# wadx2019/rpo

Measured on AMD Instinct MI355X. Metric: env-steps/sec (whole node), SafeCartpole-v0 (CartSafe-v0) RPODDPG, rollout + one batch-256 constrained policy update per vector step, higher is better.
Workload: dtype f32; 1 GPU; CartSafe-v0 RPODDPG, 4096 vectorised envs per MI355X, scripts/cart_exp.py hyper-parameters, update batch 256 every vector step (reference cadence), replay capacity 20000 per env; envs_per_gpu=4096, global_envs=4096, update_batch=256, hip_graph=True, training_batch_projection=row-wise, rccl_ranks=0, collectives_in_graph=False, graphs_replayed_on_all_ranks=True, graph_capture_fell_back_to_eager=False

## Files before the change

### include/rpo_hip.h

```cpp
#ifndef RPO_HIP_H
#define RPO_HIP_H

#ifdef __cplusplus
extern "C" {
#endif

#define RPO_ABI_VERSION 6

#define RPO_ERR_ARG (-1)
#define RPO_ERR_NULL (-2)

#define RPO_CART_STATE_DIM 6
#define RPO_CART_ACTION_DIM 2
#define RPO_CART_INEQ 6
#define RPO_CART_ROW 24
#define RPO_CART_RING 32
#define RPO_CART_CONSTS_LEN 35

#define RPO_PEND_INTERNAL_DIM 4
#define RPO_PEND_OBS_DIM 5
#define RPO_PEND_ACTION_DIM 2
#define RPO_PEND_ROW 16
#define RPO_PEND_RING 16

// ... 355 lines not shown
int rpo_evopf_reset(int n_envs, float* state, int* ep_len, float* ep_ret, const unsigned* ep_count,
                    const float* consts_dev, unsigned long long seed, unsigned env_id_base, void* stream);

int rpo_evopf_step(int n_envs, float* state, const float* action, int* ep_len, float* ep_ret, unsigned* ep_count,
                   float* rows, long long cap_steps, float* stats, int stats_cap, long long* ctrl, int max_episode_steps,
                   int auto_reset, float viol_thresh, const float* consts_dev, unsigned long long seed,
                   unsigned env_id_base, void* stream);

int rpo_evopf_act_project(int n, const float* state, int state_stride, const float* ap_raw, const float* noise, float* action, int* iters,
                          int noise_mode, int ap_is_raw, float eps_start, float eps_end, float eps_decay, int max_steps,
                          float corr_lr, float corr_eps, float corr_momentum, float newton_tol, int newton_max_iters,
                          const float* consts_dev, unsigned long long seed, unsigned env_id_base, const long long* ctrl,
                          float* stats, int stats_cap, void* stream);

int rpo_evopf_tanh_box_bwd(int n, const float* state, int state_stride, const float* raw, const float* noise,
                           float eps_start, float eps_end, float eps_decay, const long long* ctrl, const float* dap,
                           float* dout, const float* consts_dev, void* stream);

int rpo_evopf_gauss_head(int n, const float* state, int state_stride, const float* raw, const float* eps, int deterministic,
                         float* ap_out, float* logp_out, const float* consts_dev, void* stream);
int rpo_evopf_gauss_head_bwd(int n, const float* state, int state_stride, const float* raw, const float* eps,
                             const float* dap, float dlogp, float* draw, const float* consts_dev, void* stream);

int rpo_evopf_complete_bwd(int n, const float* action, const float* grad_action, const float* grad_action_b, const float* grad_action2,
                           float* grad_ap, const float* consts_dev, void* stream);

int rpo_evopf_resid(int n, const float* state, int state_stride, const float* action, float* eq_out, float* ineq_out,
                    const float* consts_dev, void* stream);

int rpo_evopf_ineq_partial_grad(int n, const float* state, int state_stride, const float* action, float* step_out, const float* consts_dev,
                                void* stream);

int rpo_evopf_eq_vjp(int n, const float* action, const float* grad_eq, float* grad_action, int autograd_sign,
                     const float* consts_dev, void* stream);

int rpo_evopf_lagrangian(int n, const float* state, int state_stride, const float* action, const float* nu, float scale, float* loss_out,
                         float* grad_action, float* grad_nu, const float* consts_dev, int overwrite, void* stream);


int rpo_cartsafe_rollout(const rpo_mlp* actor_host, int gauss, float scale, float base, int n_envs, float* state,
                         float* action, int* ep_len, float* ep_ret, unsigned* ep_count, float* rows, long long cap_steps,
                         float* stats, int stats_cap, long long* ctrl, int noise_mode, float eps_start, float eps_end,
                         float eps_decay, float box_lo, float box_hi, int max_steps, float corr_lr, float corr_eps,
                         float corr_momentum, const float* consts_host, int partial, int max_episode_steps,
                         int auto_reset, float viol_thresh, unsigned long long seed, unsigned env_id_base, int defer_clock,
                         void* stream);
int rpo_pendulum_rollout(const rpo_mlp* actor_host, int gauss, float scale, float base, int n_envs, float* internal,
                         float* obs, float* action, int* ep_len, float* ep_ret, unsigned* ep_count, float* rows,
                         long long cap_steps, float* stats, int stats_cap, long long* ctrl, int noise_mode,
                         float eps_start, float eps_end, float eps_decay, float box_lo, float box_hi, int max_steps,
                         float corr_lr, float corr_eps, float corr_momentum, int max_episode_steps, int auto_reset,
                         float viol_thresh, unsigned long long seed, unsigned env_id_base, int defer_clock, void* stream);

int rpo_cartsafe_evaluate(const rpo_mlp* actor_host, int gauss, float scale, float base, int n_envs, float* state,
                          float* action, int* ep_len, float* ep_ret, unsigned* ep_count, long long* ctrl, float* acc, int t0,
                          int steps, float box_lo, float box_hi, int max_steps, float corr_lr, float corr_eps,
                          float corr_momentum, const float* consts_host, int partial, int max_episode_steps,
                          float viol_thresh, void* stream);
int rpo_pendulum_evaluate(const rpo_mlp* actor_host, int gauss, float scale, float base, int n_envs, float* internal,
                          float* obs, float* action, int* ep_len, float* ep_ret, unsigned* ep_count, long long* ctrl,
                          float* acc, int t0, int steps, float box_lo, float box_hi, int max_steps, float corr_lr,
                          float corr_eps, float corr_momentum, int max_episode_steps, float viol_thresh, void* stream);

int rpo_eval_accumulate(int n, const float* rows, int row_stride, int reward_col, int done_col, int eq_col, int eq_num,
                        int ineq_col, int ineq_num, const int* iters, int step, float viol_thresh, float* acc, void* stream);

int rpo_eval_summarize(int n, const float* acc, const long long* ctrl, double* row_out, double* ws, void* stream);

int rpo_cartsafe_ddpg_critic_forward(const rpo_mlp* actor_target_host, const rpo_mlp* critic_target_host,
                                     const rpo_mlp* critic_host, float scale, float base, const float* rows,
                                     long long cap_steps, int n_envs, int batch, float* batch_out, long long* idx_out,
                                     const long long* idx_in, unsigned long long seed, unsigned sample_salt,
                                     const long long* ctrl, int max_steps, float corr_lr, float corr_eps,
                                     float corr_momentum, float box_lo, float box_hi, const float* consts_host,
                                     int partial, float* q_out, float* qn_out, float* x0_save, float* h1_save,
                                     void* stream);

int rpo_ddpg_actor_forward(int env, const rpo_mlp* actor_host, const rpo_mlp* critic_host, float scale, float base,
                                    float box_lo, float box_hi, float eps_start, float eps_end, float eps_decay,
                                    const float* batch, int batch_size, const float* noise_in, unsigned long long seed,
                                    unsigned noise_id_base, unsigned noise_salt, const long long* ctrl, const float* nu,
                                    const float* consts_host, int partial, float* ap_det, float* noise_out,
                                    float* actions, float* q_out, float* dq_out, float* g_act, float* partial_out,
                                    float* actor_x0, float* actor_h1, float* critic_x0, float* critic_h1, void* stream);
int rpo_ddpg_actor_backward(int env, const rpo_mlp* actor_host, const rpo_mlp_grad* actor_grad_host,
                                     const rpo_mlp* critic_host, int shared_embedding, const float* batch,
                                     int batch_size, const float* actions, const float* g_act, const float* ap_det,
                                     const float* noise, const float* dq, float eps_start, float eps_end,
                                     float eps_decay, float box_lo, float box_hi, float scale, float base,
                                     const long long* ctrl, const float* consts_host, int partial,
                                     const float* actor_x0, const float* actor_h1, const float* critic_x0,
                                     const float* critic_h1, float* actor_dh, float* actor_dx0, float* critic_dh,
                                     float* critic_dx0, float* da, float* dout, const float* partial_in, float* lag_out,
                                     float* nu_grad, float* gradmax, void* stream);

int rpo_sac_actor_forward(int env, const rpo_mlp* actor_host, const rpo_mlp* critic1_host, const rpo_mlp* critic2_host,
                          float scale, float base, float box_lo, float box_hi, float alpha, const float* batch,
                          int batch_size, const float* noise_in, unsigned long long seed, unsigned noise_id_base,
                          unsigned noise_salt, const long long* ctrl, const float* nu, const float* consts_host,
                          int partial, float* raw, float* noise_out, float* logp, float* actions, float* dq1, float* dq2,
                          float* g_act, float* partial_out, float* actor_x0, float* actor_h1, float* critic1_x0,
                          float* critic1_h1, float* critic2_x0, float* critic2_h1, void* stream);
int rpo_sac_actor_backward(int env, const rpo_mlp* actor_host, const rpo_mlp_grad* actor_grad_host,
                           const rpo_mlp* critic1_host, const rpo_mlp* critic2_host, int shared_embedding,
                           const float* batch, int batch_size, const float* actions, const float* g_act, const float* raw,
                           const float* noise, const float* logp, float* dq1, float* dq2, float dlogp, float box_lo,
// ... 53 lines not shown
```

### rpo_amd/csrc/fused.hip

```cpp
#include <stdlib.h>

#include <type_traits>

#include "cartsafe_dev.h"
#include "heads_dev.h"
#include "mlp_bwd.h"
#include "mlp_tile.h"
#include "pendulum_dev.h"
#include "rollout_args.h"
#include "rollout_env.h"

namespace {

using namespace rpo_mlp_dev;
using rpo_cart_dev::ActArgs;
using rpo_cart_dev::CartConsts;
using rpo_cart_dev::cart_explore_project;
using rpo_cart_dev::load_consts;

Mlp to_dev(const rpo_mlp* h) {
    return Mlp{h->Ws, h->bs, h->Wa, h->ba, h->W0, h->b0, h->W1, h->b1, h->W1b, h->b1b, h->S, h->A, h->E, h->H, h->n_out, h->cat, h->head_dim};
}


#ifndef RPO_ROLLOUT_SKIP
#define RPO_ROLLOUT_SKIP 0
#endif

template <class ENV, int EIN, int H, int RT>
__global__ __launch_bounds__(kFwdThreads) void rollout_kernel(RolloutArgs<ENV> p, typename ENV::Consts c) {
    typedef TileLds<EIN, RT, 8, 8> Lds;
    __shared__ Lds lds;
    constexpr int kInS = Lds::kS;
    constexpr int kLanes = rpo_mlp_dev::kRows * RT;
    constexpr int kStats = 10;
    const int row0 = blockIdx.x * kLanes;
    const int tid = threadIdx.x;
    const int n = p.step.n;
    const long long t = p.step.ctrl ? p.step.ctrl[RPO_CTRL_T] : 0;
    RpoEpisode ep{0, 0.0f, 0u};
    if (tid < kLanes && row0 + tid < n) ep = ENV::episode(p.step, row0 + tid);
    ENV::stage_obs(p.step, row0, kLanes, lds.in_s, kInS);
    float draw = 0.0f;
    const bool philox_noise = !p.gauss && p.act.noise_mode == RPO_NOISE_PHILOX;
    if (!(RPO_ROLLOUT_SKIP & 8) && tid < kLanes && row0 + tid < n && (p.gauss || philox_noise)) {
        const rpo_u4 u = p.gauss ? rpo_philox(p.act.seed, p.act.env_id_base + (uint32_t)(row0 + tid), (uint32_t)t, RPO_STREAM_POLICY,
                                              (uint32_t)p.step.ctrl[RPO_CTRL_UPDATES])
                                 : rpo_philox(p.act.seed, p.act.env_id_base + (uint32_t)(row0 + tid), (uint32_t)t, RPO_STREAM_ACT);
        draw = rpo_normal(u.x, u.y);
    }
    if (RPO_ROLLOUT_SKIP & 1) {
        if (tid < 2 * kLanes) lds.out[tid] = 0.25f;
        __syncthreads();
    } else {
        mlp_tile_forward<EIN, H, RT, Lds>(p.actor, lds, row0, n, nullptr, nullptr, p.gauss ? 0 : 1, p.scale, p.base);
    }

    float st[kStats];
#pragma unroll
    for (int k = 0; k < kStats; ++k) st[k] = 0.0f;
    float iters_f = 0.0f;
    const int i = row0 + tid;
    if (tid < kLanes && i < n) {
        const float eps_t = fmaxf(p.act.eps_end, p.act.eps_start - p.act.eps_decay * (float)t);
        float ap = lds.out[tid * 2];
        if (p.gauss) {
            ap = rpo_head_dev::gauss_head_row(ap, lds.out[tid * 2 + 1], draw, p.scale, p.base, p.act.box_lo, p.act.box_hi, 0, nullptr);
        }
        int k;
        typename ENV::ActArgs act = p.act;
        if (philox_noise) {
            ap = rpo_explore_clip(ap, eps_t, draw, p.act.box_lo, p.act.box_hi);
            act.noise_mode = RPO_NOISE_NONE;
        }
        float2 a;
        if (RPO_ROLLOUT_SKIP & 2) { a = make_float2(ap, 0.5f * ap); k = 0; }
        else a = ENV::project(act, c, lds.in_s + tid * kInS, i, ap, eps_t, t, k);
        iters_f = (float)k;
        reinterpret_cast<float2*>(p.act.action)[i] = a;
        const long long ring_base = p.step.rows ? (t % p.step.cap_steps) * (long long)n : 0;
        if (!(RPO_ROLLOUT_SKIP & 4)) ENV::lane(p.step, c, i, lds.in_s + tid * kInS, a, ep, ring_base, st);
    }
    if (RPO_ROLLOUT_SKIP & 16) return;
    if (p.step.stats && tid < 64) {
        float* srow = rpo_stats_row(p.step.stats, p.step.stats_cap, t);
        const int slot[kStats + 1] = {RPO_STAT_REWARD_SUM, RPO_STAT_EPISODES, RPO_STAT_RETURN_SUM, RPO_STAT_LENGTH_SUM,
                                      RPO_STAT_MAX_INEQ_SUM, RPO_STAT_MAX_EQ_SUM, RPO_STAT_VIOL_COUNT, RPO_STAT_TERMINATED,
                                      RPO_STAT_MAX_INEQ_MAX, RPO_STAT_MAX_EQ_MAX, RPO_STAT_PROJ_ITERS};
        float red[kStats + 1];
#pragma unroll
        for (int k = 0; k < kStats; ++k) red[k] = st[k];
        red[kStats] = iters_f;
        if (kLanes <= 16) rpo_row16_reduce_many(red, 3u << 8);
        else rpo_wave_reduce_many<kStats + 1, 32>(red, 3u << 8);
        rpo_stats_commit(red, 3u << 8, slot, srow);
    }
    if (!p.defer_clock) rpo_step_epilogue(p.step.ctrl, t, p.step.stats, p.step.stats_cap);
}

template <class ENV>
int launch_rollout(const RolloutArgs<ENV>& args, const typename ENV::Consts& c, int n_envs, void* stream) {
    {
        const int sel = rpo_tune(RPO_TUNE_ROLLOUT_WIDE);
        if (sel == 3 || sel == 4 || (sel == 2 && n_envs >= RPO_ROLLOUT_STREAM_FROM)) {
            const int e = rpo_rollout_stream_launch(std::is_same<ENV, CartEnv>::value ? 0 : 1, &args, &c, n_envs, stream);
            if (e >= 0) return e;
        }
    }
    const int wide_sel = rpo_tune(RPO_TUNE_ROLLOUT_WIDE);
    const int E = args.actor.E;
    const bool wide = E == 128 && (wide_sel == 0 || wide_sel == 1 ? wide_sel != 0 : n_envs >= 64 * 192);
    if (E == 128 && wide) {
        hipLaunchKernelGGL((rollout_kernel<ENV, 128, 256, 4>), dim3((n_envs + 63) / 64), dim3(kFwdThreads), 0,
                           (hipStream_t)stream, args, c);
    } else if (E == 128) {
        hipLaunchKernelGGL((rollout_kernel<ENV, 128, 256, 1>), dim3((n_envs + 15) / 16), dim3(kFwdThreads), 0,
                           (hipStream_t)stream, args, c);
    } else if (E == 256) {
        hipLaunchKernelGGL((rollout_kernel<ENV, 256, 256, 1>), dim3((n_envs + 15) / 16), dim3(kFwdThreads), 0,
                           (hipStream_t)stream, args, c);
    } else {
        return RPO_ERR_ARG;
    }
    RPO_LAUNCH_CHECK();
    return 0;
}

int check_actor(const Mlp& actor, int obs_dim, int gauss) {
    if (actor.hd > 1 || actor.S != obs_dim || actor.A != 0 || actor.n_out != (gauss ? 2 : 1) || actor.cat || actor.H != 256 || !actor.Ws ||
        !actor.W0 || !actor.W1 || (gauss && !actor.W1b))
        return RPO_ERR_ARG;
    return 0;
}

struct CriticFwdArgs {
    Mlp actor_target, critic_target, critic;
    float scale, base;
    const float* rows;
    long long cap_steps;
    int n_envs;
    int batch;
    float* batch_out;
    long long* idx_out;
    const long long* idx_in;
    uint64_t seed;
    uint32_t salt;
    const long long* ctrl;
    int max_steps; float corr_lr, corr_eps, corr_momentum, box_lo, box_hi;
    float* q_out;
    float* qn_out;
    float* x0_save; float* h1_save;
};

template <int EIN, int H>
__global__ __launch_bounds__(kFwdThreads) void cart_ddpg_critic_forward_kernel(CriticFwdArgs p, CartConsts c) {
    __shared__ TileLds<EIN> lds;
    __shared__ __attribute__((aligned(16))) float4 tile[kRows * 6];
    const int row0 = blockIdx.x * kRows;
    const int tid = threadIdx.x;
    const int B = p.batch;
    const long long t = p.ctrl[RPO_CTRL_T];
    if (tid < kRows * 6) {
        const int r = tid / 6, ch = tid - r * 6;
        float4 v = make_float4(0.0f, 0.0f, 0.0f, 0.0f);
        if (row0 + r < B) {
            long long row;
            if (p.idx_in) {
                row = p.idx_in[row0 + r];
            } else {
                const unsigned long long n_valid = (unsigned long long)((t < p.cap_steps ? t : p.cap_steps) * (long long)p.n_envs);
                const rpo_u4 u = rpo_philox(p.seed, (uint32_t)(row0 + r), (uint32_t)t + p.salt, RPO_STREAM_SAMPLE,
                                            (uint32_t)p.ctrl[RPO_CTRL_UPDATES]);
                row = (long long)__umul64hi(((unsigned long long)u.x << 32) | u.y, n_valid);
            }
            v = reinterpret_cast<const float4*>(p.rows)[row * (RPO_CART_RING / 4) + ch];
            if (blockIdx.y == 0) {
// ... 530 lines not shown
        const float2 r = reinterpret_cast<const float2*>(p.raw)[i];
        reinterpret_cast<float2*>(p.dout)[i] = rpo_head_dev::gauss_head_bwd_row(r.x, r.y, p.noise[i], dap, p.dlogp, p.scale,
                                                                                p.base, p.box_lo, p.box_hi);
    }
    __syncthreads();
    mlp_bwd_rows_body<EIN, H>(p.actor);
    if (p.shared_embedding) {
        __syncthreads();
        for (int idx = tid; idx < kRows * EIN; idx += kThreads) {
            const int r = idx / EIN, e = idx - r * EIN;
            if (row0 + r < B) {
                const size_t o = (size_t)(row0 + r) * EIN + e;
                p.actor.dx0[o] += p.critic1.dx0[o] + p.critic2.dx0[o];
            }
        }
    }
    if (blockIdx.x == 0 && tid < 7) {
        float sacc = 0.0f;
        for (int g = 0; g < p.n_parts; ++g) sacc += p.partial[g * 8 + tid];
        const float inv_b = 1.0f / (float)B;
        if (tid == 0) p.lag_out[0] = inv_b * sacc;
        else if (tid - 1 < p.n_ineq) p.nu_grad[tid - 1] += inv_b * sacc;
    }
}

}

extern "C" {

int rpo_cartsafe_rollout(const rpo_mlp* actor_host, int gauss, float scale, float base, int n_envs, float* state,
                         float* action, int* ep_len, float* ep_ret, unsigned* ep_count, float* rows, long long cap_steps,
                         float* stats, int stats_cap, long long* ctrl, int noise_mode, float eps_start, float eps_end,
                         float eps_decay, float box_lo, float box_hi, int max_steps, float corr_lr, float corr_eps,
                         float corr_momentum, const float* consts_host, int partial, int max_episode_steps,
                         int auto_reset, float viol_thresh, unsigned long long seed, unsigned env_id_base, int defer_clock,
                         void* stream) {
    if (!actor_host) return RPO_ERR_NULL;
    if (n_envs <= 0 || max_episode_steps <= 0 || max_steps < 0) return RPO_ERR_ARG;
    if (noise_mode != RPO_NOISE_NONE && noise_mode != RPO_NOISE_PHILOX && noise_mode != RPO_NOISE_CLIP_ONLY) return RPO_ERR_ARG;
    if (!state || !action || !ep_len || !ep_ret || !ep_count || !ctrl) return RPO_ERR_NULL;
    if ((rows && cap_steps <= 0) || (stats && stats_cap <= 0)) return RPO_ERR_ARG;
    RolloutArgs<CartEnv> args{};
    args.actor = to_dev(actor_host);
    if (int e = check_actor(args.actor, 6, gauss)) return e;
    CartConsts c;
    if (int e = load_consts(c, consts_host, partial)) return e;
    args.scale = scale; args.base = base; args.gauss = gauss; args.defer_clock = defer_clock ? 1 : 0;
    args.act = rpo_cart_dev::ActArgs{n_envs, nullptr, nullptr, action, nullptr, noise_mode, eps_start, eps_end, eps_decay,
                                     box_lo, box_hi, max_steps, corr_lr, corr_eps, corr_momentum, (uint64_t)seed,
                                     (uint32_t)env_id_base, ctrl, stats, stats_cap};
    args.step = rpo_cart_dev::StepArgs{n_envs, state, action, ep_len, ep_ret, ep_count, rows, cap_steps, stats, stats_cap,
                                       ctrl, max_episode_steps, auto_reset, viol_thresh, (uint64_t)seed,
                                       (uint32_t)env_id_base, 0};
    return launch_rollout<CartEnv>(args, c, n_envs, stream);
}

int rpo_pendulum_rollout(const rpo_mlp* actor_host, int gauss, float scale, float base, int n_envs, float* internal,
                         float* obs, float* action, int* ep_len, float* ep_ret, unsigned* ep_count, float* rows,
                         long long cap_steps, float* stats, int stats_cap, long long* ctrl, int noise_mode,
                         float eps_start, float eps_end, float eps_decay, float box_lo, float box_hi, int max_steps,
                         float corr_lr, float corr_eps, float corr_momentum, int max_episode_steps, int auto_reset,
                         float viol_thresh, unsigned long long seed, unsigned env_id_base, int defer_clock, void* stream) {
    if (!actor_host) return RPO_ERR_NULL;
    if (n_envs <= 0 || max_episode_steps <= 0 || max_steps < 0) return RPO_ERR_ARG;
    if (noise_mode != RPO_NOISE_NONE && noise_mode != RPO_NOISE_PHILOX && noise_mode != RPO_NOISE_CLIP_ONLY) return RPO_ERR_ARG;
    if (!internal || !action || !ep_len || !ep_ret || !ep_count || !ctrl) return RPO_ERR_NULL;
    if ((rows && cap_steps <= 0) || (stats && stats_cap <= 0)) return RPO_ERR_ARG;
    RolloutArgs<PendEnv> args{};
    args.actor = to_dev(actor_host);
    if (int e = check_actor(args.actor, 5, gauss)) return e;
    args.scale = scale; args.base = base; args.gauss = gauss; args.defer_clock = defer_clock ? 1 : 0;
    args.act = rpo_pend_dev::ActArgs{n_envs, nullptr, 5, nullptr, nullptr, action, nullptr, noise_mode, eps_start, eps_end,
                                     eps_decay, box_lo, box_hi, max_steps, corr_lr, corr_eps, corr_momentum, (uint64_t)seed,
                                     (uint32_t)env_id_base, ctrl, stats, stats_cap};
    args.step = rpo_pend_dev::StepArgs{n_envs, internal, obs, action, ep_len, ep_ret, ep_count, rows, cap_steps, stats,
                                       stats_cap, ctrl, max_episode_steps, auto_reset, viol_thresh, (uint64_t)seed,
                                       (uint32_t)env_id_base};
    return launch_rollout<PendEnv>(args, PendEnv::Consts{0}, n_envs, stream);
}

int rpo_cartsafe_ddpg_critic_forward(const rpo_mlp* actor_target_host, const rpo_mlp* critic_target_host,
                                     const rpo_mlp* critic_host, float scale, float base, const float* rows,
                                     long long cap_steps, int n_envs, int batch, float* batch_out, long long* idx_out,
                                     const long long* idx_in, unsigned long long seed, unsigned sample_salt,
                                     const long long* ctrl, int max_steps, float corr_lr, float corr_eps,
                                     float corr_momentum, float box_lo, float box_hi, const float* consts_host,
                                     int partial, float* q_out, float* qn_out, float* x0_save, float* h1_save,
                                     void* stream) {
    if (!actor_target_host || !critic_target_host || !critic_host) return RPO_ERR_NULL;
    if (batch <= 0 || cap_steps <= 0 || n_envs <= 0 || max_steps < 0) return RPO_ERR_ARG;
    if (!rows || !batch_out || !ctrl || !q_out || !qn_out || !x0_save || !h1_save) return RPO_ERR_NULL;
    CriticFwdArgs a{};
    a.actor_target = to_dev(actor_target_host); a.critic_target = to_dev(critic_target_host); a.critic = to_dev(critic_host);
    const Mlp& at = a.actor_target;
    const Mlp& ct = a.critic_target;
    const Mlp& cr = a.critic;
    if (at.S != 6 || at.A != 0 || at.n_out != 1 || at.cat || ct.S != 6 || ct.A != 2 || ct.cat || cr.S != 6 || cr.A != 2 || cr.cat ||
        at.H != 256 || ct.H != 256 || cr.H != 256 || at.E != ct.E || at.E != cr.E || ct.n_out != 1 || cr.n_out != 1)
        return RPO_ERR_ARG;
    CartConsts c;
    if (int e = load_consts(c, consts_host, partial)) return e;
    a.scale = scale; a.base = base; a.rows = rows; a.cap_steps = cap_steps; a.n_envs = n_envs; a.batch = batch;
    a.batch_out = batch_out; a.idx_out = idx_out; a.idx_in = idx_in; a.seed = (uint64_t)seed; a.salt = (uint32_t)sample_salt;
    a.ctrl = ctrl; a.max_steps = max_steps; a.corr_lr = corr_lr; a.corr_eps = corr_eps; a.corr_momentum = corr_momentum;
    a.box_lo = box_lo; a.box_hi = box_hi; a.q_out = q_out; a.qn_out = qn_out; a.x0_save = x0_save; a.h1_save = h1_save;
    const int grid = (batch + kRows - 1) / kRows;
// ... 378 lines not shown
```

### rpo_amd/csrc/mlp_tile.h

```cpp
#pragma once
#include "common.h"

namespace rpo_mlp_dev {

typedef float f32x4 __attribute__((ext_vector_type(4)));

constexpr int kRows = 16;
constexpr int kThreads = 256;
constexpr int kFwdWaves = 8;
constexpr int kFwdThreads = kFwdWaves * 64;
constexpr int kInS = 64, kInA = 48;

struct Mlp {
    const float *Ws, *bs, *Wa, *ba, *W0, *b0, *W1, *b1, *W1b, *b1b;
    int S, A, E, H, n_out, cat;
    int hd;
    int l1_vec;
};
struct MlpGrad {
    float *Ws, *bs, *Wa, *ba, *W0, *b0, *W1, *b1, *W1b, *b1b;
};

__device__ __forceinline__ f32x4 mfma4(float a, float b, f32x4 c) {
    return __builtin_amdgcn_mfma_f32_16x16x4f32(a, b, c, 0, 0, 0);
}

template <int EIN, int RT = 1, int INS = kInS, int INA = kInA>
struct TileLds {
    static constexpr int ROWS = kRows * RT;
    static constexpr int kS = INS, kA = INA;
    __attribute__((aligned(16))) float x1[ROWS * (EIN + 4)];
    float in_s[ROWS * INS];
    float in_a[ROWS * INA];
    float part[kFwdWaves * ROWS * 2];
    float out[ROWS * 2];
};

constexpr int kWideOut = 32;

template <int EIN, int H>
struct TileLdsWide : TileLds<EIN, 1, kInS, kInA> {
    __attribute__((aligned(16))) float hr[kRows * (H + 4)];
    float outw[kRows * kWideOut];
};

template <int EIN, int H, int RT>
struct TileWeights {
    static constexpr int NT = H / (16 * kFwdWaves);
    static constexpr int ITS = EIN / 16;
    static constexpr int PRE_MAX = RT > 1 ? 4 : 16;
    static constexpr int PRE = ITS < PRE_MAX ? ITS : PRE_MAX;
    static constexpr int TPW = EIN / (16 * kFwdWaves);
    float bias;
    float ws0[8], wa0[8];
    float wk[TPW][3];
    float4 wpre[PRE][NT];
    float b0v[NT], w1av[NT], w1bv[NT];
    float b1v;
};

template <int EIN>
__device__ __forceinline__ bool tile_l1_mfma(const Mlp& net) {
    return EIN == 128 && !net.cat && net.S <= 6 && net.A <= 4 && net.S > 0 && !net.l1_vec;
}

#ifndef RPO_TILE_SKIP
#define RPO_TILE_SKIP 0
#endif

template <int EIN, int H, int RT>
__device__ __forceinline__ void tile_load_weights(const Mlp& net, TileWeights<EIN, H, RT>& w) {
    constexpr int ROWS = kRows * RT;
    constexpr int NT = TileWeights<EIN, H, RT>::NT, PRE = TileWeights<EIN, H, RT>::PRE;
    const int tid = threadIdx.x, lane = tid & 63, wave = tid >> 6;
    const int li = lane & 15, lg = lane >> 4;
    if (RPO_TILE_SKIP & 1) {
        w.bias = 0.01f * (float)li;
#pragma unroll
        for (int u = 0; u < 8; ++u) { w.ws0[u] = 0.1f; w.wa0[u] = 0.1f; }
#pragma unroll
        for (int it = 0; it < PRE; ++it)
#pragma unroll
            for (int c = 0; c < NT; ++c) w.wpre[it][c] = make_float4(0.01f, -0.01f, 0.02f, 0.01f * (float)lg);
#pragma unroll
        for (int c = 0; c < NT; ++c) { w.b0v[c] = 0.1f; w.w1av[c] = 0.05f; w.w1bv[c] = 0.0f; }
        w.b1v = 0.0f;
        return;
    }
    if (tile_l1_mfma<EIN>(net)) {
        constexpr int TPW = TileWeights<EIN, H, RT>::TPW;
        const bool add_a = net.A > 0;
        w.bias = 0.0f;
#pragma unroll
        for (int t = 0; t < TPW; ++t) {
            const int e = (wave + t * kFwdWaves) * 16 + li;
            const float* p0 = lg == 0 ? net.bs + e : (lg == 1 ? net.ba + e : net.Ws + e * net.S + (lg - 2));
            const bool live0 = lg == 0 || (lg == 1 ? add_a : lg - 2 < net.S);
            w.wk[t][0] = live0 ? *p0 : 0.0f;
            w.wk[t][1] = 2 + lg < net.S ? net.Ws[e * net.S + 2 + lg] : 0.0f;
            w.wk[t][2] = (add_a && lg < net.A) ? net.Wa[e * net.A + lg] : 0.0f;
        }
    } else {
        const int e_col = tid % EIN;
        const bool act_part = net.cat && e_col >= net.E;
        const int er = act_part ? e_col - net.E : e_col;
        const bool use_s = !act_part, use_a = net.A > 0 && (act_part || !net.cat);
        w.bias = act_part ? net.ba[er] : (net.bs[er] + ((net.A > 0 && !net.cat) ? net.ba[er] : 0.0f));
#pragma unroll
        for (int u = 0; u < 8; ++u) {
            w.ws0[u] = (use_s && u < net.S) ? net.Ws[er * net.S + u] : 0.0f;
            w.wa0[u] = (use_a && u < net.A) ? net.Wa[er * net.A + u] : 0.0f;
        }
    }
    const int j0 = wave * (H / kFwdWaves);
#pragma unroll
// ... 223 lines not shown
```

### rpo_amd/csrc/rollout_args.h

```cpp
#pragma once
#include "mlp_tile.h"
#include "rollout_env.h"

namespace {

using rpo_mlp_dev::Mlp;

template <class ENV>
struct RolloutArgs {
    Mlp actor;
    float scale, base;
    int gauss;
    int defer_clock;
    typename ENV::ActArgs act;
    typename ENV::StepArgs step;
};

}

__attribute__((visibility("hidden"))) int rpo_rollout_stream_launch(int env , const void* args,
                                                                    const void* consts, int n_envs, void* stream);
```

### rpo_amd/csrc/train_ops.hip

```cpp
#include <stdlib.h>
#include "common.h"
#include "heads_dev.h"

namespace {

__global__ __launch_bounds__(RPO_BLOCK) void td_huber_kernel(
    int n, const float* __restrict__ q1, const float* __restrict__ q2, const float* __restrict__ qn1,
    const float* __restrict__ qn2, const float* __restrict__ logp, float alpha, const float* __restrict__ reward,
    int reward_stride, const float* __restrict__ done, int done_stride, float gamma, float* __restrict__ loss_out,
    float* __restrict__ grad_q1, float* __restrict__ grad_q2, float* __restrict__ target_out) {
    __shared__ float red[RPO_BLOCK / RPO_WAVE];
    const float inv_n = 1.0f / (float)n;
    float acc = 0.0f;
    for (int i = blockIdx.x * RPO_BLOCK + threadIdx.x; i < n; i += gridDim.x * RPO_BLOCK) {
        const float qn = rpo_head_dev::td_next_value(qn1[i], qn2 ? qn2[i] : 0.0f, qn2 != nullptr,
                                                     logp ? logp[i] : 0.0f, logp != nullptr, alpha);
        const float y = rpo_head_dev::td_target(reward[(size_t)i * reward_stride], done[(size_t)i * done_stride], gamma,
                                                qn);
        if (target_out) target_out[i] = y;
        float h1 = 0.0f, h2 = 0.0f;
        const float g1 = rpo_head_dev::td_huber_row(q1[i], y, inv_n, &h1);
        if (grad_q1) grad_q1[i] = g1;
        if (q2) {
            const float g2 = rpo_head_dev::td_huber_row(q2[i], y, inv_n, &h2);
            if (grad_q2) grad_q2[i] = g2;
        }
        acc += h1 + h2;
    }
    const float r = rpo_wave_sum(acc);
    if ((threadIdx.x & (RPO_WAVE - 1)) == 0) red[threadIdx.x / RPO_WAVE] = r;
    __syncthreads();
    if (threadIdx.x == 0 && loss_out) {
        float s = 0.0f;
        for (int w = 0; w < RPO_BLOCK / RPO_WAVE; ++w) s += red[w];
        atomicAdd(loss_out, s);
    }
}

__global__ __launch_bounds__(RPO_BLOCK) void absmax_kernel(long long n, const float* __restrict__ x,
                                                           float* __restrict__ max_out, int slotted) {
    __shared__ float red[RPO_BLOCK / RPO_WAVE];
    float m = 0.0f;
    const long long n4 = n / 4;
    const float4* x4 = reinterpret_cast<const float4*>(x);
    for (long long i = (long long)blockIdx.x * RPO_BLOCK + threadIdx.x; i < n4; i += (long long)gridDim.x * RPO_BLOCK) {
        const float4 v = x4[i];
        m = fmaxf(fmaxf(m, fabsf(v.x)), fmaxf(fabsf(v.y), fmaxf(fabsf(v.z), fabsf(v.w))));
    }
    for (long long i = n4 * 4 + (long long)blockIdx.x * RPO_BLOCK + threadIdx.x; i < n; i += (long long)gridDim.x * RPO_BLOCK)
        m = fmaxf(m, fabsf(x[i]));
    m = rpo_wave_max(m);
    if ((threadIdx.x & (RPO_WAVE - 1)) == 0) red[threadIdx.x / RPO_WAVE] = m;
    __syncthreads();
    if (threadIdx.x == 0) {
        for (int w = 1; w < RPO_BLOCK / RPO_WAVE; ++w) m = fmaxf(m, red[w]);
        m = fmaxf(m, red[0]);
        float* dst = slotted ? max_out + (blockIdx.x % RPO_GRADMAX_SLOTS) * (RPO_GRADMAX_LEN / RPO_GRADMAX_SLOTS) : max_out;
        if (m > 0.0f) rpo_atomic_max_nonneg(dst, m);
    }
}

struct AdamArgs {
    long long n;
    float* param;
    float* grad;
    float* m;
    float* v;
    int* step_dev;
    float lr, beta1, beta2, eps, weight_decay;
    int maximize;
    float clip_thres;
    float* gradmax;
    int reset_gradmax;
    int zero_grad;
    int clamp_min0;
    float* target;
    float tau;
    long long* arrive;
    float* target2;
    long long n2;
    int polyak_only;
    long long* clock;
    int prepared;
};

__device__ __forceinline__ void adam_body(const AdamArgs& p) {
    if (p.polyak_only) {
        for (long long i = (long long)blockIdx.x * RPO_BLOCK + threadIdx.x; i < p.n; i += (long long)gridDim.x * RPO_BLOCK)
            p.target[i] = p.target[i] * (1.0f - p.tau) + p.param[i] * p.tau;
        return;
    }
    const long long i0 = (long long)blockIdx.x * RPO_BLOCK + threadIdx.x, stride = (long long)gridDim.x * RPO_BLOCK;
    float g0 = 0.0f, w0 = 0.0f, m0 = 0.0f, v0 = 0.0f, t0 = 0.0f, t20 = 0.0f;
    if (i0 < p.n) {
        g0 = p.grad[i0]; w0 = p.param[i0]; m0 = p.m[i0]; v0 = p.v[i0];
        if (p.target) t0 = p.target[i0];
        if (p.target2 && i0 < p.n2) t20 = p.target2[i0];
    }
    asm volatile("" ::: "memory");
    float gm = 0.0f;
    if (p.clip_thres > 0.0f) {
#pragma unroll
        for (int j = 0; j < RPO_GRADMAX_SLOTS; ++j) gm = fmaxf(gm, p.gradmax[j * (RPO_GRADMAX_LEN / RPO_GRADMAX_SLOTS)]);
    }
    const int step = p.prepared ? p.step_dev[0] : p.step_dev[0] + 1;
    double* cache = reinterpret_cast<double*>(p.step_dev + 4);
    double bc1 = cache[0], bc2s = cache[1];
    if (bc1 == 0.0 || p.step_dev[1] != step) {
        bc1 = 1.0 - pow((double)p.beta1, (double)step);
        bc2s = sqrt(1.0 - pow((double)p.beta2, (double)step));
    }
    const float step_size = (float)((double)p.lr / bc1);
    const float bc2_sqrt = (float)bc2s;
    const float coef = p.clip_thres > 0.0f ? fminf(p.clip_thres / (gm + 1e-6f), 1.0f) : 1.0f;
    const float omb1 = 1.0f - p.beta1, omb2 = 1.0f - p.beta2;
    for (long long i = i0; i < p.n; i += stride) {
        if (i != i0) {
            g0 = p.grad[i]; w0 = p.param[i]; m0 = p.m[i]; v0 = p.v[i];
            if (p.target) t0 = p.target[i];
            if (p.target2 && i < p.n2) t20 = p.target2[i];
        }
        float g = g0 * coef;
        if (p.zero_grad) p.grad[i] = 0.0f;
        else if (p.clip_thres > 0.0f) p.grad[i] = g;
        if (p.maximize) g = -g;
        float w = w0;
        if (p.weight_decay != 0.0f) g += p.weight_decay * w;
        float m = m0, v = v0;
        m = m + (g - m) * omb1;
        v = v * p.beta2 + omb2 * g * g;
        const float denom = sqrtf(v) / bc2_sqrt + p.eps;
        w = w - step_size * (m / denom);
        if (p.clamp_min0) w = fmaxf(w, 0.0f);
        p.param[i] = w; p.m[i] = m; p.v[i] = v;
        if (p.target) p.target[i] = t0 * (1.0f - p.tau) + w * p.tau;
        if (p.target2 && i < p.n2) p.target2[i] = t20 * (1.0f - p.tau) + w * p.tau;
    }
    if (p.prepared) return;
    __syncthreads();
    if (threadIdx.x == 0) {
        const unsigned n = gridDim.x, sub = blockIdx.x % 16u;
        unsigned long long* top = reinterpret_cast<unsigned long long*>(p.arrive);
        bool last;
        if (n <= 16u) {
            last = atomicAdd(top, 1ull) == (unsigned long long)n - 1ull;
        } else {
            unsigned long long* sc = reinterpret_cast<unsigned long long*>(p.step_dev + 32 + 32 * sub);
            const unsigned long long in_sub = (n - sub + 15u) / 16u;
            last = false;
            if (atomicAdd(sc, 1ull) == in_sub - 1ull) {
                *sc = 0;
                last = atomicAdd(top, 1ull) == 15ull;
            }
        }
        if (last) {
            *top = 0;
            p.step_dev[0] = step;
            cache[0] = 1.0 - pow((double)p.beta1, (double)(step + 1));
            cache[1] = sqrt(1.0 - pow((double)p.beta2, (double)(step + 1)));
            p.step_dev[1] = step + 1;
            if (p.reset_gradmax && p.gradmax)
                for (int j = 0; j < RPO_GRADMAX_SLOTS; ++j) p.gradmax[j * (RPO_GRADMAX_LEN / RPO_GRADMAX_SLOTS)] = 0.0f;
            if (p.clock) p.clock[0] += 1;
        }
    }
}

__global__ __launch_bounds__(RPO_BLOCK) void adam_kernel(AdamArgs p) { adam_body(p); }

struct AdamArgs4 {
    AdamArgs seg[4];
};
__global__ __launch_bounds__(RPO_BLOCK) void adam_multi_kernel(AdamArgs4 p) { adam_body(p.seg[blockIdx.y]); }

__global__ __launch_bounds__(RPO_BLOCK) void min_q_bwd_kernel(int n, const float* __restrict__ q1, const float* __restrict__ q2,
                                                              float scale, float* __restrict__ dq1, float* __restrict__ dq2) {
    for (int i = blockIdx.x * RPO_BLOCK + threadIdx.x; i < n; i += gridDim.x * RPO_BLOCK) {
        const float a = q1[i], b = q2[i];
        const float w = (a < b ? 1.0f : 0.0f) + 0.5f * (a == b ? 1.0f : 0.0f);
        dq1[i] = w * scale;
        dq2[i] = (1.0f - w) * scale;
    }
}

__global__ __launch_bounds__(RPO_BLOCK) void polyak_kernel(long long n, const float* __restrict__ param,
                                                           float* __restrict__ target, float tau) {
// ... 152 lines not shown
```

Baseline: 102.1 million env-steps/s.

## Fuse actor Adam step into CartSafe rollout kernel with in-register first-layer update

New measurement: 101.1 million env-steps/s. -1.0%, worse.

```diff
diff --git a/include/rpo_hip.h b/include/rpo_hip.h
--- a/include/rpo_hip.h
+++ b/include/rpo_hip.h
@@ -431,6 +431,28 @@
                          float corr_lr, float corr_eps, float corr_momentum, int max_episode_steps, int auto_reset,
                          float viol_thresh, unsigned long long seed, unsigned env_id_base, int defer_clock, void* stream);
 
+#define RPO_ADAM_RIDE_SYNC_LEN 96
+#define RPO_ADAM_RIDE_GAVE_UP 64
+typedef struct rpo_adam_ride {
+    long long n;
+    float *param, *grad, *exp_avg, *exp_avg_sq;
+    int* step_dev;
+    float lr, beta1, beta2, eps, weight_decay;
+    int maximize;
+    float clip_thres;
+    float* gradmax;
+    int zero_grad, clamp_min0;
+    long long emb_lo, emb_hi;
+    unsigned* sync;
+} rpo_adam_ride;
+int rpo_cartsafe_rollout_adam(const rpo_mlp* actor_host, int gauss, float scale, float base, int n_envs, float* state,
+                              float* action, int* ep_len, float* ep_ret, unsigned* ep_count, float* rows, long long cap_steps,
+                              float* stats, int stats_cap, long long* ctrl, int noise_mode, float eps_start, float eps_end,
+                              float eps_decay, float box_lo, float box_hi, int max_steps, float corr_lr, float corr_eps,
+                              float corr_momentum, const float* consts_host, int partial, int max_episode_steps,
+                              int auto_reset, float viol_thresh, unsigned long long seed, unsigned env_id_base, int defer_clock,
+                              const rpo_adam_ride* ride, void* stream);
+
 int rpo_cartsafe_evaluate(const rpo_mlp* actor_host, int gauss, float scale, float base, int n_envs, float* state,
                           float* action, int* ep_len, float* ep_ret, unsigned* ep_count, long long* ctrl, float* acc, int t0,
                           int steps, float box_lo, float box_hi, int max_steps, float corr_lr, float corr_eps,
diff --git a/rpo_amd/csrc/adam_elem.h b/rpo_amd/csrc/adam_elem.h
--- /dev/null
+++ b/rpo_amd/csrc/adam_elem.h
@@ -0,0 +1,57 @@
+#pragma once
+#include "common.h"
+
+namespace rpo_adam_dev {
+
+struct AdamScalars {
+    float coef;
+    float step_size;
+    float bc2_sqrt;
+    float omb1, omb2;
+};
+
+template <bool CACHED_ONLY = false>
+__device__ __forceinline__ AdamScalars adam_scalars(const float* gradmax, const int* step_dev, int prepared, float lr, float beta1,
+                                                    float beta2, float clip_thres, int* step_out, bool* cached = nullptr) {
+    float gm = 0.0f;
+    if (clip_thres > 0.0f) {
+#pragma unroll
+        for (int j = 0; j < RPO_GRADMAX_SLOTS; ++j) gm = fmaxf(gm, gradmax[j * (RPO_GRADMAX_LEN / RPO_GRADMAX_SLOTS)]);
+    }
+    const int step = prepared ? step_dev[0] : step_dev[0] + 1;
+    const double* cache = reinterpret_cast<const double*>(step_dev + 4);
+    double bc1 = cache[0], bc2s = cache[1];
+    const bool miss = bc1 == 0.0 || step_dev[1] != step;
+    if (cached) *cached = !miss;
+    if constexpr (!CACHED_ONLY) {
+        if (miss) {
+            bc1 = 1.0 - pow((double)beta1, (double)step);
+            bc2s = sqrt(1.0 - pow((double)beta2, (double)step));
+        }
+    }
+    AdamScalars s;
+    s.step_size = (float)((double)lr / bc1);
+    s.bc2_sqrt = (float)bc2s;
+    s.coef = clip_thres > 0.0f ? fminf(clip_thres / (gm + 1e-6f), 1.0f) : 1.0f;
+    s.omb1 = 1.0f - beta1;
+    s.omb2 = 1.0f - beta2;
+    *step_out = step;
+    return s;
+}
+
+__device__ __forceinline__ float adam_element(const AdamScalars& s, float g0, float w0, float& m, float& v, float beta2, float eps,
+                                              float weight_decay, int maximize, int clamp_min0, float* g_clipped) {
+    float g = g0 * s.coef;
+    *g_clipped = g;
+    if (maximize) g = -g;
+    float w = w0;
+    if (weight_decay != 0.0f) g += weight_decay * w;
+    m = m + (g - m) * s.omb1;
+    v = v * beta2 + s.omb2 * g * g;
+    const float denom = sqrtf(v) / s.bc2_sqrt + eps;
+    w = w - s.step_size * (m / denom);
+    if (clamp_min0) w = fmaxf(w, 0.0f);
+    return w;
+}
+
+}
diff --git a/rpo_amd/csrc/fused.hip b/rpo_amd/csrc/fused.hip
--- a/rpo_amd/csrc/fused.hip
+++ b/rpo_amd/csrc/fused.hip
@@ -2,6 +2,7 @@
 
 #include <type_traits>
 
+#include "adam_elem.h"
 #include "cartsafe_dev.h"
 #include "heads_dev.h"
 #include "mlp_bwd.h"
@@ -27,10 +28,96 @@
 #define RPO_ROLLOUT_SKIP 0
 #endif
 
-template <class ENV, int EIN, int H, int RT>
-__global__ __launch_bounds__(kFwdThreads) void rollout_kernel(RolloutArgs<ENV> p, typename ENV::Consts c) {
+struct RideRegs {
+    float g[2], m[2], v[2];
+    bool in[2];
+};
+
+template <int EIN>
+__device__ __forceinline__ void ride_request(const AdamRide& r, const Mlp& net, RideRegs& rr) {
+    const int tid = threadIdx.x, lane = tid & 63, wave = tid >> 6;
+    const int li = lane & 15, lg = lane >> 4;
+    const int e = wave * 16 + li;
+    const float* q[2];
+    q[0] = lg == 0 ? net.bs + e : net.Ws + e * net.S + (lg - 2);
+    q[1] = net.Ws + e * net.S + 2 + lg;
+    const bool live[2] = {lg == 0 || (lg >= 2 && lg - 2 < net.S), 2 + lg < net.S};
+#pragma unroll
+    for (int k = 0; k < 2; ++k) {
+        const long long idx = q[k] - r.param;
+        rr.in[k] = live[k] && idx >= r.emb_lo && idx < r.emb_hi;
+        rr.g[k] = rr.m[k] = rr.v[k] = 0.0f;
+        if (rr.in[k]) { rr.g[k] = r.grad[idx]; rr.m[k] = r.m[idx]; rr.v[k] = r.v[idx]; }
+    }
+}
+
+template <int EIN, int H, int RT>
+__device__ __forceinline__ void ride_apply(const AdamRide& r, const RideRegs& rr, TileWeights<EIN, H, RT>& w) {
+    int step;
+    bool cached;
+    const rpo_adam_dev::AdamScalars sc = rpo_adam_dev::adam_scalars<true>(r.gradmax, r.step_dev, 1, r.lr, r.beta1, r.beta2,
+                                                                          r.clip_thres, &step, &cached);
+#pragma unroll
+    for (int k = 0; k < 2; ++k) {
+        float m = rr.m[k], v = rr.v[k], g;
+        const float stepped = rpo_adam_dev::adam_element(sc, rr.g[k], w.wk[0][k], m, v, r.beta2, r.eps, r.weight_decay, r.maximize,
+                                                         r.clamp_min0, &g);
+        if (rr.in[k]) w.wk[0][k] = stepped;
+    }
+    asm volatile("s_waitcnt vmcnt(0)" ::: "memory");
+    __syncthreads();
+    if (threadIdx.x == 0) {
+        __hip_atomic_fetch_add(r.sync + kRideReaders, 1u, __ATOMIC_RELAXED, __HIP_MEMORY_SCOPE_AGENT);
+        if (!cached) __hip_atomic_store(r.sync + kRideGaveUp, 1u, __ATOMIC_RELAXED, __HIP_MEMORY_SCOPE_AGENT);
+    }
+}
+
+__device__ __forceinline__ void ride_adam_plane(const AdamRide& r, int b) {
+    const long long i = (long long)b * kFwdThreads + threadIdx.x;
+    const long long lo = (long long)b * kFwdThreads, hi = lo + kFwdThreads;
+    const bool overlaps = lo < r.emb_hi && hi > r.emb_lo && r.emb_lo < r.emb_hi;
+    float g0 = 0.0f, w0 = 0.0f, m = 0.0f, v = 0.0f;
+    if (i < r.n) { g0 = r.grad[i]; w0 = r.param[i]; m = r.m[i]; v = r.v[i]; }
+    int step;
+    const rpo_adam_dev::AdamScalars sc = rpo_adam_dev::adam_scalars(r.gradmax, r.step_dev, 1, r.lr, r.beta1, r.beta2, r.clip_thres,
+                                                                    &step);
+    float g;
+    const float w = rpo_adam_dev::adam_element(sc, g0, w0, m, v, r.beta2, r.eps, r.weight_decay, r.maximize, r.clamp_min0, &g);
+    if (overlaps) {
+        if (threadIdx.x == 0) {
+            int polls = 0;
+            while (__hip_atomic_fetch_add(r.sync + kRideReaders, 0u, __ATOMIC_RELAXED, __HIP_MEMORY_SCOPE_AGENT) < (unsigned)r.n_roll) {
+                if (++polls >= kRideSpinMax) {
+                    __hip_atomic_store(r.sync + kRideGaveUp, 1u, __ATOMIC_RELAXED, __HIP_MEMORY_SCOPE_AGENT);
+                    break;
+                }
+                __builtin_amdgcn_s_sleep(1);
+            }
+        }
+        __syncthreads();
+    }
+    if (i < r.n) {
+        if (r.zero_grad) r.grad[i] = 0.0f;
+        else if (r.clip_thres > 0.0f) r.grad[i] = g;
+        r.param[i] = w; r.m[i] = m; r.v[i] = v;
+    }
+    if (overlaps && threadIdx.x == 0) {
+        const long long first = r.emb_lo / kFwdThreads, last = (r.emb_hi - 1) / kFwdThreads;
+        const unsigned n_over = (unsigned)(last - first + 1);
+        if (__hip_atomic_fetch_add(r.sync + kRideArrive, 1u, __ATOMIC_RELAXED, __HIP_MEMORY_SCOPE_AGENT) == n_over - 1u) {
+            __hip_atomic_store(r.sync + kRideReaders, 0u, __ATOMIC_RELAXED, __HIP_MEMORY_SCOPE_AGENT);
+            __hip_atomic_store(r.sync + kRideArrive, 0u, __ATOMIC_RELAXED, __HIP_MEMORY_SCOPE_AGENT);
+        }
+    }
+}
+
+template <class ENV, int EIN, int H, int RT, bool RIDE>
+__device__ __forceinline__ void rollout_body(const RolloutArgs<ENV>& p, const typename ENV::Consts& c, const AdamRide* ride) {
     typedef TileLds<EIN, RT, 8, 8> Lds;
     __shared__ Lds lds;
+    if constexpr (RIDE) {
+        if ((int)blockIdx.x >= ride->n_roll) { ride_adam_plane(*ride, (int)blockIdx.x - ride->n_roll); return; }
+    }
     constexpr int kInS = Lds::kS;
     constexpr int kLanes = rpo_mlp_dev::kRows * RT;
     constexpr int kStats = 10;
@@ -53,7 +140,17 @@
         if (tid < 2 * kLanes) lds.out[tid] = 0.25f;
         __syncthreads();
     } else {
-        mlp_tile_forward<EIN, H, RT, Lds>(p.actor, lds, row0, n, nullptr, nullptr, p.gauss ? 0 : 1, p.scale, p.base);
+        if constexpr (RIDE) {
+            static_assert(EIN == 128 && RT == 1, "the ride recomputes the matrix-core form's first-layer operands");
+            TileWeights<EIN, H, RT> w;
+            RideRegs rr;
+            ride_request<EIN>(*ride, p.actor, rr);
+            tile_load_weights<EIN, H, RT>(p.actor, w);
+            ride_apply<EIN, H, RT>(*ride, rr, w);
+            tile_compute<EIN, H, RT, Lds>(p.actor, w, lds, row0, n, nullptr, nullptr, p.gauss ? 0 : 1, p.scale, p.base);
+        } else {
+            mlp_tile_forward<EIN, H, RT, Lds>(p.actor, lds, row0, n, nullptr, nullptr, p.gauss ? 0 : 1, p.scale, p.base);
+        }
     }
 
     float st[kStats];
@@ -95,7 +192,19 @@
         else rpo_wave_reduce_many<kStats + 1, 32>(red, 3u << 8);
         rpo_stats_commit(red, 3u << 8, slot, srow);
     }
-    if (!p.defer_clock) rpo_step_epilogue(p.step.ctrl, t, p.step.stats, p.step.stats_cap);
+    if constexpr (!RIDE) {
+        if (!p.defer_clock) rpo_step_epilogue(p.step.ctrl, t, p.step.stats, p.step.stats_cap);
+    }
+}
+
+template <class ENV, int EIN, int H, int RT>
+__global__ __launch_bounds__(kFwdThreads) void rollout_kernel(RolloutArgs<ENV> p, typename ENV::Consts c) {
+    rollout_body<ENV, EIN, H, RT, false>(p, c, nullptr);
+}
+
+template <class ENV>
+__global__ __launch_bounds__(kFwdThreads) void rollout_adam_kernel(RolloutArgs<ENV> p, typename ENV::Consts c, AdamRide ride) {
+    rollout_body<ENV, 128, 256, 1, true>(p, c, &ride);
 }
 
 template <class ENV>
@@ -122,6 +231,18 @@
     } else {
         return RPO_ERR_ARG;
     }
+    RPO_LAUNCH_CHECK();
+    return 0;
+}
+
+template <class ENV>
+int launch_rollout_adam(const RolloutArgs<ENV>& args, const typename ENV::Consts& c, int n_envs, const AdamRide& ride, void* stream) {
+    const int sel = rpo_tune(RPO_TUNE_ROLLOUT_WIDE);
+    const bool row16 = sel == 0 || (sel == 2 && n_envs < 64 * 192 && n_envs < RPO_ROLLOUT_STREAM_FROM);
+    if (!row16 || args.actor.E != 128 || !tile_l1_mfma<128>(args.actor)) return -1;
+    const int writers = (int)((ride.n + kFwdThreads - 1) / kFwdThreads);
+    hipLaunchKernelGGL((rollout_adam_kernel<ENV>), dim3(ride.n_roll + writers), dim3(kFwdThreads), 0, (hipStream_t)stream, args, c,
+                       ride);
     RPO_LAUNCH_CHECK();
     return 0;
 }
@@ -758,6 +879,50 @@
     args.step = rpo_cart_dev::StepArgs{n_envs, state, action, ep_len, ep_ret, ep_count, rows, cap_steps, stats, stats_cap,
                                        ctrl, max_episode_steps, auto_reset, viol_thresh, (uint64_t)seed,
                                        (uint32_t)env_id_base, 0};
+    return launch_rollout<CartEnv>(args, c, n_envs, stream);
+}
+
+int rpo_cartsafe_rollout_adam(const rpo_mlp* actor_host, int gauss, float scale, float base, int n_envs, float* state,
+                              float* action, int* ep_len, float* ep_ret, unsigned* ep_count, float* rows, long long cap_steps,
+                              float* stats, int stats_cap, long long* ctrl, int noise_mode, float eps_start, float eps_end,
+                              float eps_decay, float box_lo, float box_hi, int max_steps, float corr_lr, float corr_eps,
+                              float corr_momentum, const float* consts_host, int partial, int max_episode_steps,
+                              int auto_reset, float viol_thresh, unsigned long long seed, unsigned env_id_base, int defer_clock,
+                              const rpo_adam_ride* ride, void* stream) {
+    if (!ride)
+        return rpo_cartsafe_rollout(actor_host, gauss, scale, base, n_envs, state, action, ep_len, ep_ret, ep_count, rows, cap_steps,
+                                    stats, stats_cap, ctrl, noise_mode, eps_start, eps_end, eps_decay, box_lo, box_hi, max_steps,
+                                    corr_lr, corr_eps, corr_momentum, consts_host, partial, max_episode_steps, auto_reset,
+                                    viol_thresh, seed, env_id_base, defer_clock, stream);
+    if (!actor_host) return RPO_ERR_NULL;
+    if (n_envs <= 0 || max_episode_steps <= 0 || max_steps < 0) return RPO_ERR_ARG;
+    if (noise_mode != RPO_NOISE_NONE && noise_mode != RPO_NOISE_PHILOX && noise_mode != RPO_NOISE_CLIP_ONLY) return RPO_ERR_ARG;
+    if (!state || !action || !ep_len || !ep_ret || !ep_count || !ctrl) return RPO_ERR_NULL;
+    if ((rows && cap_steps <= 0) || (stats && stats_cap <= 0)) return RPO_ERR_ARG;
+    if (ride->n <= 0 || ride->emb_lo < 0 || ride->emb_hi <= ride->emb_lo || ride->emb_hi > ride->n || !defer_clock) return RPO_ERR_ARG;
+    if (!ride->param || !ride->grad || !ride->exp_avg || !ride->exp_avg_sq || !ride->step_dev || !ride->sync) return RPO_ERR_NULL;
+    if (ride->clip_thres > 0.0f && !ride->gradmax) return RPO_ERR_NULL;
+    RolloutArgs<CartEnv> args{};
+    args.actor = to_dev(actor_host);
+    if (int e = check_actor(args.actor, 6, gauss)) return e;
+    CartConsts c;
+    if (int e = load_consts(c, consts_host, partial)) return e;
+    args.scale = scale; args.base = base; args.gauss = gauss; args.defer_clock = 1;
+    args.act = rpo_cart_dev::ActArgs{n_envs, nullptr, nullptr, action, nullptr, noise_mode, eps_start, eps_end, eps_decay,
+                                     box_lo, box_hi, max_steps, corr_lr, corr_eps, corr_momentum, (uint64_t)seed,
+                                     (uint32_t)env_id_base, ctrl, stats, stats_cap};
+    args.step = rpo_cart_dev::StepArgs{n_envs, state, action, ep_len, ep_ret, ep_count, rows, cap_steps, stats, stats_cap,
+                                       ctrl, max_episode_steps, auto_reset, viol_thresh, (uint64_t)seed,
+                                       (uint32_t)env_id_base, 0};
+    AdamRide r{ride->n, ride->param, ride->grad, ride->exp_avg, ride->exp_avg_sq, ride->step_dev, ride->gradmax, ride->lr,
+               ride->beta1, ride->beta2, ride->eps, ride->weight_decay, ride->clip_thres, ride->maximize ? 1 : 0,
+               ride->zero_grad ? 1 : 0, ride->clamp_min0 ? 1 : 0, ride->emb_lo, ride->emb_hi, ride->sync, (n_envs + 15) / 16};
+    const int e = launch_rollout_adam<CartEnv>(args, c, n_envs, r, stream);
+    if (e >= 0) return e;
+    if (int e2 = rpo_adam_step(ride->n, ride->param, ride->grad, ride->exp_avg, ride->exp_avg_sq, ride->step_dev, ride->lr,
+                               ride->beta1, ride->beta2, ride->eps, ride->weight_decay, ride->maximize, ride->clip_thres,
+                               ride->gradmax, 0, ride->zero_grad, ride->clamp_min0, nullptr, 0.0f, nullptr, 1, stream))
+        return e2;
     return launch_rollout<CartEnv>(args, c, n_envs, stream);
 }
 
diff --git a/rpo_amd/csrc/mlp_tile.h b/rpo_amd/csrc/mlp_tile.h
--- a/rpo_amd/csrc/mlp_tile.h
+++ b/rpo_amd/csrc/mlp_tile.h
@@ -60,7 +60,7 @@
 };
 
 template <int EIN>
-__device__ __forceinline__ bool tile_l1_mfma(const Mlp& net) {
+__host__ __device__ __forceinline__ bool tile_l1_mfma(const Mlp& net) {
     return EIN == 128 && !net.cat && net.S <= 6 && net.A <= 4 && net.S > 0 && !net.l1_vec;
 }
 
diff --git a/rpo_amd/csrc/rollout_args.h b/rpo_amd/csrc/rollout_args.h
--- a/rpo_amd/csrc/rollout_args.h
+++ b/rpo_amd/csrc/rollout_args.h
@@ -5,6 +5,20 @@
 namespace {
 
 using rpo_mlp_dev::Mlp;
+
+struct AdamRide {
+    long long n;
+    float *param, *grad, *m, *v;
+    const int* step_dev;
+    const float* gradmax;
+    float lr, beta1, beta2, eps, weight_decay, clip_thres;
+    int maximize, zero_grad, clamp_min0;
+    long long emb_lo, emb_hi;
+    unsigned* sync;
+    int n_roll;
+};
+constexpr int kRideReaders = 0, kRideArrive = 32, kRideGaveUp = 64;
+constexpr int kRideSpinMax = 1 << 18;
 
 template <class ENV>
 struct RolloutArgs {
diff --git a/rpo_amd/csrc/train_ops.hip b/rpo_amd/csrc/train_ops.hip
--- a/rpo_amd/csrc/train_ops.hip
+++ b/rpo_amd/csrc/train_ops.hip
@@ -1,4 +1,5 @@
 #include <stdlib.h>
+#include "adam_elem.h"
 #include "common.h"
 #include "heads_dev.h"
 
@@ -98,40 +99,20 @@
         if (p.target2 && i0 < p.n2) t20 = p.target2[i0];
     }
     asm volatile("" ::: "memory");
-    float gm = 0.0f;
-    if (p.clip_thres > 0.0f) {
-#pragma unroll
-        for (int j = 0; j < RPO_GRADMAX_SLOTS; ++j) gm = fmaxf(gm, p.gradmax[j * (RPO_GRADMAX_LEN / RPO_GRADMAX_SLOTS)]);
-    }
-    const int step = p.prepared ? p.step_dev[0] : p.step_dev[0] + 1;
+    int step;
+    const rpo_adam_dev::AdamScalars sc = rpo_adam_dev::adam_scalars(p.gradmax, p.step_dev, p.prepared, p.lr, p.beta1, p.beta2,
+                                                                    p.clip_thres, &step);
     double* cache = reinterpret_cast<double*>(p.step_dev + 4);
-    double bc1 = cache[0], bc2s = cache[1];
-    if (bc1 == 0.0 || p.step_dev[1] != step) {
-        bc1 = 1.0 - pow((double)p.beta1, (double)step);
-        bc2s = sqrt(1.0 - pow((double)p.beta2, (double)step));
-    }
-    const float step_size = (float)((double)p.lr / bc1);
-    const float bc2_sqrt = (float)bc2s;
-    const float coef = p.clip_thres > 0.0f ? fminf(p.clip_thres / (gm + 1e-6f), 1.0f) : 1.0f;
-    const float omb1 = 1.0f - p.beta1, omb2 = 1.0f - p.beta2;
     for (long long i = i0; i < p.n; i += stride) {
         if (i != i0) {
             g0 = p.grad[i]; w0 = p.param[i]; m0 = p.m[i]; v0 = p.v[i];
             if (p.target) t0 = p.target[i];
             if (p.target2 && i < p.n2) t20 = p.target2[i];
         }
-        float g = g0 * coef;
+        float m = m0, v = v0, g;
+        const float w = rpo_adam_dev::adam_element(sc, g0, w0, m, v, p.beta2, p.eps, p.weight_decay, p.maximize, p.clamp_min0, &g);
         if (p.zero_grad) p.grad[i] = 0.0f;
         else if (p.clip_thres > 0.0f) p.grad[i] = g;
-        if (p.maximize) g = -g;
-        float w = w0;
-        if (p.weight_decay != 0.0f) g += p.weight_decay * w;
-        float m = m0, v = v0;
-        m = m + (g - m) * omb1;
-        v = v * p.beta2 + omb2 * g * g;
-        const float denom = sqrtf(v) / bc2_sqrt + p.eps;
-        w = w - step_size * (m / denom);
-        if (p.clamp_min0) w = fmaxf(w, 0.0f);
         p.param[i] = w; p.m[i] = m; p.v[i] = v;
         if (p.target) p.target[i] = t0 * (1.0f - p.tau) + w * p.tau;
         if (p.target2 && i < p.n2) p.target2[i] = t20 * (1.0f - p.tau) + w * p.tau;
```
